# rwl/CSparse.py

Measured on AMD Instinct MI355X. Metric: cs_gaxpy achieved HBM GB/s (algorithmic bytes / time), 5M x 5M CSC, 64 nnz/col, higher is better.
Workload: dtype f64; 1 GPU; cs_gaxpy y += A x on G-rand: 5000000 x 5000000 CSC, 64 distinct rows per column drawn uniformly from [0, n), ascending (SURVEY 8d), int32 indices, fp64 values; one independent matrix per GPU; row_draw=uniform, n=5000000, nnz=320000000, kernel=gaxpy_tiled, plan_key_bytes=3, parallelism=independent matrices, 1 per GPU, no data-path collective

## Files before the change

csparse.py_amd/csrc/csx_gaxpy_tiled.hip:

```cpp
#include <cstdlib>

#include "csx_internal.h"

namespace csx {

constexpr int TL_WAVES = 4, TL_NG = 5;
constexpr int TL_GROUP = 256;
constexpr int TL_LDS_BYTES = 160 * 1024 - 256;
constexpr int TL_LDS_ROWS = TL_LDS_BYTES / 8 - 2;
typedef uint32_t u32x4 __attribute__((ext_vector_type(4)));
typedef double f64x2 __attribute__((ext_vector_type(2)));

__global__ __launch_bounds__(256) void k_tile_keys(int64_t nnz, const int32_t *__restrict__ Ai,
                                                   const int32_t *__restrict__ col, int rb_bits, int32_t row_block,
                                                   int32_t slab_cols, int32_t nslab, uint32_t *__restrict__ tile_id,
                                                   uint32_t *__restrict__ packed) {
    int64_t p = (int64_t)blockIdx.x * blockDim.x + threadIdx.x;
    if (p >= nnz) return;
    const uint32_t i = (uint32_t)Ai[p], j = (uint32_t)col[p];
    const uint32_t s = j / (uint32_t)slab_cols, lc = j - s * (uint32_t)slab_cols;
    const uint32_t b = i / (uint32_t)row_block, lr = i - b * (uint32_t)row_block;
    tile_id[p] = b * (uint32_t)nslab + s;
    packed[p] = (lc << rb_bits) | lr;
}

__global__ __launch_bounds__(256) void k_padded_lengths(int64_t ntiles, const int32_t *__restrict__ sptr,
                                                        int32_t *__restrict__ ngroups) {
    int64_t t = (int64_t)blockIdx.x * blockDim.x + threadIdx.x;
    if (t < ntiles) ngroups[t] = (sptr[t + 1] - sptr[t] + TL_GROUP - 1) / TL_GROUP;
}

__global__ __launch_bounds__(256) void k_group_info(int64_t ntiles, int32_t nslab, const int32_t *__restrict__ sptr,
                                                    const int32_t *__restrict__ gptr, uint32_t *__restrict__ info) {
    int64_t t = (int64_t)blockIdx.x * blockDim.x + threadIdx.x;
    if (t >= ntiles) return;
    const int32_t len = sptr[t + 1] - sptr[t];
    const uint32_t slab = (uint32_t)(t % nslab);
    int32_t g = gptr[t];
    for (int32_t left = len; left > 0; left -= TL_GROUP, g++) info[g] = (slab << 9) | (uint32_t)min(left, TL_GROUP);
}

__global__ __launch_bounds__(256) void k_interleave(int64_t nnz, const uint32_t *__restrict__ stid,
                                                    const int32_t *__restrict__ sptr, const int32_t *__restrict__ gptr,
                                                    const uint32_t *__restrict__ skey, const double *__restrict__ sval,
                                                    uint32_t *__restrict__ okey, double *__restrict__ oval) {
    int64_t q = (int64_t)blockIdx.x * blockDim.x + threadIdx.x;
    if (q >= nnz) return;
    const uint32_t t = stid[q];
    const int32_t e = (int32_t)(q - sptr[t]);
    const int32_t g = e / TL_GROUP, w = e % TL_GROUP;
    const int64_t gbase = ((int64_t)gptr[t] + g) * TL_GROUP;
    const int l = w & 63, k = w >> 6;
    if (okey) okey[gbase + l * 4 + k] = skey[q];
    oval[gbase + (k >> 1) * 128 + l * 2 + (k & 1)] = sval[q];
}

__global__ __launch_bounds__(256) void k_run_span(int64_t nnz, const uint32_t *__restrict__ stid,
                                                  const int32_t *__restrict__ sptr, const uint32_t *__restrict__ skey,
                                                  int rb_bits, int *too_wide) {
    int64_t q = (int64_t)blockIdx.x * blockDim.x + threadIdx.x;
    if (q >= nnz) return;
    const int32_t e = (int32_t)(q - sptr[stid[q]]);
    const int64_t first = q - (e & 63);
    if ((skey[q] >> rb_bits) - (skey[first] >> rb_bits) >= 512u) *too_wide = 1;
}

__global__ __launch_bounds__(256) void k_interleave24(int64_t nnz, const uint32_t *__restrict__ stid,
                                                      const int32_t *__restrict__ sptr, const int32_t *__restrict__ gptr,
                                                      const uint32_t *__restrict__ skey, int rb_bits,
                                                      uint8_t *__restrict__ okey, uint32_t *__restrict__ obase) {
    int64_t q = (int64_t)blockIdx.x * blockDim.x + threadIdx.x;
    if (q >= nnz) return;
    const uint32_t t = stid[q];
    const int32_t e = (int32_t)(q - sptr[t]);
    const int32_t g = e / TL_GROUP, w = e % TL_GROUP;
    const int l = w & 63, k = w >> 6;
    const uint32_t rmask = (1u << rb_bits) - 1u;
    const uint32_t col = skey[q] >> rb_bits, col0 = skey[q - l] >> rb_bits;
    const uint32_t v = (skey[q] & rmask) | ((col - col0) << 15);
    const int64_t gg = (int64_t)gptr[t] + g;
    uint8_t *o = okey + gg * (TL_GROUP * 3) + l * 12 + k * 3;
    o[0] = (uint8_t)v;
    o[1] = (uint8_t)(v >> 8);
    o[2] = (uint8_t)(v >> 16);
    if (l == 0) obase[gg * 4 + k] = col;
}

__global__ __launch_bounds__(256) void k_fill_key24(uint8_t *p, int64_t nslots, uint32_t v) {
    int64_t i = (int64_t)blockIdx.x * blockDim.x + threadIdx.x;
    const int64_t stride = (int64_t)gridDim.x * blockDim.x;
    for (; i < nslots; i += stride) {
        p[3 * i] = (uint8_t)v;
        p[3 * i + 1] = (uint8_t)(v >> 8);
        p[3 * i + 2] = (uint8_t)(v >> 16);
    }
}

__global__ __launch_bounds__(256) void k_fill_keys(uint32_t *p, int64_t n, uint32_t v) {
    int64_t i = (int64_t)blockIdx.x * blockDim.x + threadIdx.x;
    const int64_t stride = (int64_t)gridDim.x * blockDim.x;
    for (; i < n; i += stride) p[i] = v;
}

struct GroupRegs {
    u32x4 kk;
    u32x4 base;
    f64x2 v0, v1;
    uint32_t info;
};

template <bool NT, bool K24>
__device__ __forceinline__ GroupRegs load_group_t(const uint32_t *__restrict__ key, const double *__restrict__ val,
                                                  const uint32_t *__restrict__ info, const uint32_t *__restrict__ base,
                                                  int32_t g, int lane) {
    GroupRegs r;
    const int64_t gb = (int64_t)g * TL_GROUP;
    if (K24) {
        const uint32_t *kp = key + (int64_t)g * (TL_GROUP * 3 / 4) + 3 * lane;
        const uint32_t ka = __builtin_nontemporal_load(kp), kb = __builtin_nontemporal_load(kp + 1),
                       kc = __builtin_nontemporal_load(kp + 2);
        r.kk.x = ka & 0xFFFFFFu;
        r.kk.y = (ka >> 24) | ((kb & 0xFFFFu) << 8);
        r.kk.z = (kb >> 16) | ((kc & 0xFFu) << 16);
        r.kk.w = kc >> 8;
        r.base = *reinterpret_cast<const u32x4 *>(base + 4 * (int64_t)g);
        r.v0 = __builtin_nontemporal_load(reinterpret_cast<const f64x2 *>(val + gb + 2 * lane));
        r.v1 = __builtin_nontemporal_load(reinterpret_cast<const f64x2 *>(val + gb + 128 + 2 * lane));
    } else if (NT) {
        r.kk = __builtin_nontemporal_load(reinterpret_cast<const u32x4 *>(key + gb + 4 * lane));
        r.v0 = __builtin_nontemporal_load(reinterpret_cast<const f64x2 *>(val + gb + 2 * lane));
        r.v1 = __builtin_nontemporal_load(reinterpret_cast<const f64x2 *>(val + gb + 128 + 2 * lane));
    } else {
        r.kk = *reinterpret_cast<const u32x4 *>(key + gb + 4 * lane);
        r.v0 = *reinterpret_cast<const f64x2 *>(val + gb + 2 * lane);
        r.v1 = *reinterpret_cast<const f64x2 *>(val + gb + 128 + 2 * lane);
    }
    r.info = info[g];
    return r;
}

template <int HOW>
__device__ __forceinline__ double load_x(const double *p) {
    if (HOW == 1) return __hip_atomic_load(p, __ATOMIC_RELAXED, __HIP_MEMORY_SCOPE_AGENT);
    if (HOW == 2) return __builtin_nontemporal_load(p);
    return *p;
}

template <int VARIANT, int NW, int NG, bool K24>
struct TiledStep {
    static constexpr bool GATHER = !(VARIANT & 1) || VARIANT >= 5, ATOMIC = VARIANT != 3;
    static constexpr bool STREAM_NT = VARIANT != 2;
    static constexpr uint32_t CMASK = VARIANT == 5 ? 32767u : (VARIANT == 4 ? 255u : 0xffffffffu);
    static constexpr int XLOAD = VARIANT == 6 ? 1 : 0;
    static constexpr bool RING = VARIANT == 7;

    static __device__ __forceinline__ void load_set(GroupRegs (&r)[NG], const uint32_t *__restrict__ key,
                                                    const double *__restrict__ val, const uint32_t *__restrict__ info,
                                                    const uint32_t *__restrict__ base, int32_t g, int32_t g0,
                                                    int32_t gend, int lane) {
#pragma unroll
        for (int j = 0; j < NG; j++) {
            int32_t gg = g + j * NW < gend ? g + j * NW : gend - 1;
            if (RING) gg = g0 + ((gg - g0) & 31);
            r[j] = load_group_t<STREAM_NT, K24>(key, val, info, base, gg, lane);
        }
    }

    static __device__ __forceinline__ void step(GroupRegs (&cur)[NG], GroupRegs (&nxt)[NG], double *ytile,
                                                const uint32_t *__restrict__ key, const double *__restrict__ val,
                                                const uint32_t *__restrict__ info, const uint32_t *__restrict__ base,
                                                const double *__restrict__ x, int32_t &g, int32_t g0, int32_t gend,
                                                int lane, int rb_bits, uint32_t rmask, int32_t slab_cols, double &sink) {
        double xv[NG][4];
#pragma unroll
        for (int j = 0; j < NG; j++) {
            xv[j][0] = xv[j][1] = xv[j][2] = xv[j][3] = 1.0;
            if (GATHER && (j == 0 || g + j * NW < gend)) {
                const double *xs = x + (int64_t)(cur[j].info >> 9) * slab_cols;
                if (K24) {
                    xv[j][0] = load_x<XLOAD>(xs + ((cur[j].base.x + (cur[j].kk.x >> 15)) & CMASK));
                    xv[j][1] = load_x<XLOAD>(xs + ((cur[j].base.y + (cur[j].kk.y >> 15)) & CMASK));
                    xv[j][2] = load_x<XLOAD>(xs + ((cur[j].base.z + (cur[j].kk.z >> 15)) & CMASK));
                    xv[j][3] = load_x<XLOAD>(xs + ((cur[j].base.w + (cur[j].kk.w >> 15)) & CMASK));
                } else {
                    xv[j][0] = load_x<XLOAD>(xs + ((cur[j].kk.x >> rb_bits) & CMASK));
                    xv[j][1] = load_x<XLOAD>(xs + ((cur[j].kk.y >> rb_bits) & CMASK));
                    xv[j][2] = load_x<XLOAD>(xs + ((cur[j].kk.z >> rb_bits) & CMASK));
                    xv[j][3] = load_x<XLOAD>(xs + ((cur[j].kk.w >> rb_bits) & CMASK));
                }
            }
        }
        load_set(nxt, key, val, info, base, g + NG * NW, g0, gend, lane);
#pragma unroll
        for (int j = 0; j < NG; j++) {
            if (j == 0 || g + j * NW < gend) {
                if (ATOMIC) {
                    unsafeAtomicAdd(&ytile[cur[j].kk.x & rmask], cur[j].v0.x * xv[j][0]);
                    unsafeAtomicAdd(&ytile[cur[j].kk.y & rmask], cur[j].v0.y * xv[j][1]);
                    unsafeAtomicAdd(&ytile[cur[j].kk.z & rmask], cur[j].v1.x * xv[j][2]);
                    unsafeAtomicAdd(&ytile[cur[j].kk.w & rmask], cur[j].v1.y * xv[j][3]);
                } else {
                    sink += cur[j].v0.x * xv[j][0] + cur[j].v0.y * xv[j][1] + cur[j].v1.x * xv[j][2] +
                            cur[j].v1.y * xv[j][3] +
                            (double)((cur[j].kk.x ^ cur[j].kk.y ^ cur[j].kk.z ^ cur[j].kk.w) & 1u);
                }
            }
        }
        g += NG * NW;
    }
};

template <int VARIANT, int NW, int NG, bool K24>
__global__ __launch_bounds__(64 * NW) void k_gaxpy_tiled(const int32_t *__restrict__ rb_gptr,
                                                         const uint32_t *__restrict__ group_info,
                                                         const uint32_t *__restrict__ tile_key,
                                                         const uint32_t *__restrict__ tile_base,
                                                         const double *__restrict__ tile_val,
                                                         const double *__restrict__ x, double *__restrict__ y,
                                                         int32_t m, int32_t nrb, int32_t row_block,
                                                         int32_t slab_cols, int rb_bits) {
    extern __shared__ __attribute__((aligned(16))) double ytile[];
    typedef TiledStep<VARIANT, NW, NG, K24> S;
    const uint32_t rmask = K24 ? 0x7FFFu : (1u << rb_bits) - 1u;
    const int lane = threadIdx.x & 63, wave = threadIdx.x >> 6;
    double sink = 0.0;
    for (int32_t rb = blockIdx.x; rb < nrb; rb += gridDim.x) {
        const int64_t row0 = (int64_t)rb * row_block;
        const int32_t rows = (int32_t)((row0 + row_block <= m) ? row_block : (m - row0));
        for (int k = threadIdx.x; k < rows; k += 64 * NW) ytile[k] = y[row0 + k];
        __syncthreads();
        const int32_t gend = rb_gptr[rb + 1];
        const int32_t g0 = rb_gptr[rb];
        int32_t g = g0 + wave;
        if (g < gend) {
            GroupRegs A[NG], B[NG];
            S::load_set(A, tile_key, tile_val, group_info, tile_base, g, g0, gend, lane);
            for (;;) {
                S::step(A, B, ytile, tile_key, tile_val, group_info, tile_base, x, g, g0, gend, lane, rb_bits, rmask, slab_cols, sink);
                if (g >= gend) break;
                S::step(B, A, ytile, tile_key, tile_val, group_info, tile_base, x, g, g0, gend, lane, rb_bits, rmask, slab_cols, sink);
                if (g >= gend) break;
            }
        }
        __syncthreads();
        if (!S::ATOMIC && sink == 12345.678) ytile[0] = sink;
        for (int k = threadIdx.x; k < rows; k += 64 * NW) y[row0 + k] = ytile[k];
        __syncthreads();
    }
}

__global__ __launch_bounds__(256) void k_rb_group_ptr(int32_t nrb, int32_t nslab, const int32_t *__restrict__ gptr,
                                                      int32_t *__restrict__ rb_gptr) {
    int64_t b = (int64_t)blockIdx.x * blockDim.x + threadIdx.x;
    if (b <= nrb) rb_gptr[b] = gptr[(int64_t)b * nslab];
}

static int gaxpy_tiled_pick_shape(Csc *A);

int gaxpy_tiled_prepare(Csc *A) {
    if (A->tiled) return CSX_OK;
    if (!A->x) return CSX_EINVAL;
    hipStream_t s = ctx().stream;
    const int32_t nwg = ctx().cus > 0 ? ctx().cus : 256;
    const int32_t cap = TL_LDS_ROWS;
    int32_t rounds = 1;
    int32_t row_block;
    for (;;) {
        const int64_t nrb_try = (int64_t)nwg * rounds;
        row_block = (int32_t)(((int64_t)A->m + nrb_try - 1) / nrb_try);
        if (row_block <= cap) break;
        rounds++;
    }
    if (row_block < 1) row_block = 1;
    const int32_t nrb = (int32_t)(((int64_t)A->m + row_block - 1) / row_block);
    int rb_bits = 1;
    while ((1 << rb_bits) <= row_block) rb_bits++;
    double slab_kb = 1024.0;
#ifdef CSX_ABLATION
    if (const char *e = std::getenv("CSX_TILED_SLAB_KB")) slab_kb = std::atof(e) >= 8.0 ? std::atof(e) : slab_kb;
#endif
    int64_t slab_cols = (int64_t)(slab_kb * 1024 / 8);
    const int64_t max_cols_key = 1ll << (32 - rb_bits);
    if (slab_cols > max_cols_key) slab_cols = max_cols_key;
    if (slab_cols > A->n) slab_cols = A->n > 0 ? A->n : 1;
    int32_t nslab = (int32_t)(((int64_t)A->n + slab_cols - 1) / slab_cols);
    if (nslab < 1) nslab = 1;
    const int64_t ntiles = (int64_t)nrb * nslab;
    if (ntiles > 0x3fffffffll || nslab >= (1 << 22)) return CSX_EINVAL;

    std::unique_ptr<TiledPlan> t(new TiledPlan());
    t->rb_bits = rb_bits;
    t->row_block = row_block;
    t->nrb = nrb;
    t->nslab = nslab;
    t->slab_cols = (int32_t)slab_cols;
    {
        DevBuf<int32_t> col, sptr, gptr;
        DevBuf<uint32_t> tid, packed, stid, skey;
        DevBuf<double> sval;
        int64_t ngroups = 0;
        CSX_TRY(col.alloc((size_t)A->nnz));
        CSX_TRY(tid.alloc((size_t)A->nnz));
        CSX_TRY(packed.alloc((size_t)A->nnz));
        CSX_TRY(stid.alloc((size_t)A->nnz));
        CSX_TRY(skey.alloc((size_t)A->nnz));
        CSX_TRY(sval.alloc((size_t)A->nnz));
        CSX_TRY(sptr.alloc((size_t)ntiles + 1));
        CSX_TRY(gptr.alloc((size_t)ntiles + 1));
        CSX_TRY(t->tile_ptr.alloc((size_t)nrb + 1));
        CSX_TRY(expand_columns(A->p, A->n, A->nnz, col));
        if (A->nnz > 0) {
            int64_t blocks = ((int64_t)A->nnz + 255) / 256;
            hipLaunchKernelGGL(k_tile_keys, dim3((unsigned)blocks), dim3(256), 0, s, (int64_t)A->nnz, A->i, col, rb_bits,
                               row_block, t->slab_cols, t->nslab, tid, packed);
            CSX_LAUNCH_CHECK();
        }
        CSX_TRY(stable_sort_by_key(tid, packed, A->x, A->nnz, (uint32_t)ntiles, stid, skey, sval));
        CSX_TRY(boundaries_from_sorted(stid, A->nnz, (int32_t)ntiles, sptr));
        const unsigned tb = (unsigned)((ntiles + 256) / 256);
        hipLaunchKernelGGL(k_padded_lengths, dim3(tb), dim3(256), 0, s, ntiles, sptr, gptr);
        CSX_TRY(scan_exclusive_i32(gptr, gptr, ntiles, &ngroups));
        bool k24 = false;
        if (ngroups > 0 && rb_bits <= 15 && ctx().opt.gaxpy_keys24) {
            DevBuf<int> flag;
            int h = 1;
            CSX_TRY(flag.alloc(1));
            (void)hipMemsetAsync(flag, 0, sizeof(int), s);
            hipLaunchKernelGGL(k_run_span, dim3((unsigned)(((int64_t)A->nnz + 255) / 256)), dim3(256), 0, s, (int64_t)A->nnz,
                               stid, sptr, skey, rb_bits, flag);
            CSX_HIP(hipMemcpyAsync(&h, flag, sizeof(int), hipMemcpyDeviceToHost, s));
            CSX_HIP(hipStreamSynchronize(s));
            k24 = h == 0;
        }
        t->ngroups = ngroups;
        CSX_TRY(t->tile_len.alloc((size_t)ngroups));
        if (!k24) CSX_TRY(t->tile_key.alloc((size_t)ngroups * TL_GROUP));
        if (k24) CSX_TRY(t->tile_key24.alloc((size_t)ngroups * TL_GROUP * 3 + 16));
        if (k24) CSX_TRY(t->tile_base.alloc((size_t)ngroups * 4));
        CSX_TRY(t->tile_val.alloc((size_t)ngroups * TL_GROUP));
        if (ngroups > 0) {
            if (k24) {
                hipLaunchKernelGGL(k_fill_key24, dim3(2048), dim3(256), 0, s, t->tile_key24, (int64_t)ngroups * TL_GROUP,
                                   (uint32_t)row_block);
                (void)hipMemsetAsync(t->tile_base, 0, (size_t)ngroups * 4 * sizeof(uint32_t), s);
            } else {
                hipLaunchKernelGGL(k_fill_keys, dim3(2048), dim3(256), 0, s, t->tile_key, (int64_t)ngroups * TL_GROUP,
                                   (uint32_t)row_block);
            }
            (void)hipMemsetAsync(t->tile_val, 0, (size_t)ngroups * TL_GROUP * sizeof(double), s);
            hipLaunchKernelGGL(k_group_info, dim3(tb), dim3(256), 0, s, ntiles, nslab, sptr, gptr, (uint32_t *)t->tile_len.get());
            hipLaunchKernelGGL(k_interleave, dim3((unsigned)(((int64_t)A->nnz + 255) / 256)), dim3(256), 0, s,
                               (int64_t)A->nnz, stid, sptr, gptr, skey, sval, t->tile_key, t->tile_val);
            if (k24)
                hipLaunchKernelGGL(k_interleave24, dim3((unsigned)(((int64_t)A->nnz + 255) / 256)), dim3(256), 0, s,
                                   (int64_t)A->nnz, stid, sptr, gptr, skey, rb_bits, t->tile_key24, t->tile_base);
        }
        hipLaunchKernelGGL(k_rb_group_ptr, dim3((unsigned)((nrb + 256) / 256)), dim3(256), 0, s, nrb, nslab, gptr,
                           t->tile_ptr);
        CSX_LAUNCH_CHECK();
        CSX_HIP(hipStreamSynchronize(s));
    }
    A->tiled = std::move(t);
#ifndef CSX_ABLATION
    if (ctx().opt.gaxpy_tune_shape) CSX_TRY(gaxpy_tiled_pick_shape(A));
#endif
    return CSX_OK;
}

constexpr int TL_NSHAPES = 4;
static int gaxpy_tiled_launch(const Csc *A, const double *x, double *y, int shape);

static int gaxpy_tiled_pick_shape(Csc *A) {
    TiledPlan *t = A->tiled.get();
    if ((int64_t)A->nnz < (int64_t)1 << 24) return CSX_OK;
    hipStream_t s = ctx().stream;
    DevBuf<double> x, y;
    if (x.alloc((size_t)A->n) != CSX_OK || y.alloc((size_t)A->m) != CSX_OK) return CSX_OK;
    CSX_HIP(hipMemsetAsync(x, 0, (size_t)A->n * sizeof(double), s));
    CSX_HIP(hipMemsetAsync(y, 0, (size_t)A->m * sizeof(double), s));
    hipEvent_t e0, e1;
    CSX_HIP(hipEventCreate(&e0));
    CSX_HIP(hipEventCreate(&e1));
    int best = 0;
    int st = CSX_OK;
    for (int round = 0; round < 2 && st == CSX_OK; round++)
        for (int sh = 0; sh < TL_NSHAPES && st == CSX_OK; sh++) {
            if (round == 0) st = gaxpy_tiled_launch(A, x, y, sh);
            if (st != CSX_OK) break;
            (void)hipEventRecord(e0, s);
            for (int rep = 0; rep < 3 && st == CSX_OK; rep++) st = gaxpy_tiled_launch(A, x, y, sh);
            (void)hipEventRecord(e1, s);
            if (hipEventSynchronize(e1) != hipSuccess) st = CSX_ERUNTIME;
            float ms = 0.f;
            (void)hipEventElapsedTime(&ms, e0, e1);
            ms /= 3;
            if (round == 0 || ms < t->shape_ms[sh]) t->shape_ms[sh] = ms;
        }
    (void)hipEventDestroy(e0);
    (void)hipEventDestroy(e1);
    if (st != CSX_OK) return st;
    for (int sh = 1; sh < TL_NSHAPES; sh++)
        if (t->shape_ms[sh] < t->shape_ms[best]) best = sh;
    t->shape = best;
    return CSX_OK;
}

int gaxpy_tiled_shape(const TiledPlan *t) {
    const int forced = ctx().opt.gaxpy_shape;
    if (forced >= 0 && forced < TL_NSHAPES) return forced;
    return t->shape >= 0 && t->shape < TL_NSHAPES ? t->shape : 0;
}

int gaxpy_tiled_run(const Csc *A, const double *x, double *y) {
    return gaxpy_tiled_launch(A, x, y, gaxpy_tiled_shape(A->tiled.get()));
}

int gaxpy_tiled_group_counts(const TiledPlan *t, std::vector<int32_t> &groups) {
    std::vector<int32_t> ptr((size_t)t->nrb + 1);
    hipStream_t s = ctx().stream;
    CSX_HIP(hipMemcpyAsync(ptr.data(), t->tile_ptr, ptr.size() * sizeof(int32_t), hipMemcpyDeviceToHost, s));
    CSX_HIP(hipStreamSynchronize(s));
    groups.resize((size_t)t->nrb);
    for (int32_t b = 0; b < t->nrb; b++) groups[b] = ptr[b + 1] - ptr[b];
    return CSX_OK;
}

static int gaxpy_tiled_launch(const Csc *A, const double *x, double *y, int shape) {
    const TiledPlan *t = A->tiled.get();
    hipStream_t s = ctx().stream;
    const size_t lds = (((size_t)(t->row_block + 1) * sizeof(double)) + 15) & ~(size_t)15;
    const int32_t nwg = ctx().cus > 0 ? ctx().cus : 256;
    const unsigned grid = (unsigned)(t->nrb < nwg ? t->nrb : nwg);
#define CSX_TILED_LAUNCH_K(V, NW, NG, K24)                                                                           \
    {                                                                                                                \
        CSX_HIP(hipFuncSetAttribute(reinterpret_cast<const void *>(&k_gaxpy_tiled<V, NW, NG, K24>),                  \
                                    hipFuncAttributeMaxDynamicSharedMemorySize, TL_LDS_BYTES));                      \
        hipLaunchKernelGGL((k_gaxpy_tiled<V, NW, NG, K24>), dim3(grid), dim3(64 * NW), lds, s, t->tile_ptr,          \
                           (const uint32_t *)t->tile_len.get(),                                                      \
                           K24 ? reinterpret_cast<const uint32_t *>(t->tile_key24.get()) : t->tile_key.get(),        \
                           t->tile_base,                                                                             \
                           t->tile_val, x, y, A->m, t->nrb, t->row_block, t->slab_cols, t->rb_bits);                 \
    }
#define CSX_TILED_LAUNCH(V, NW, NG)                                                                                  \
    {                                                                                                                \
        if (t->tile_key24) CSX_TILED_LAUNCH_K(V, NW, NG, true) else CSX_TILED_LAUNCH_K(V, NW, NG, false)             \
    }
#ifdef CSX_ABLATION
    int code = 0;
    if (const char *e = std::getenv("CSX_TILED_VARIANT")) code = std::atoi(e);
    const int v = code % 100, nw = (code / 100) % 100 ? (code / 100) % 100 : TL_WAVES, ng = code / 10000 ? code / 10000 : TL_NG;
#define CSX_V(V)                                             \
    if (v == V) {                                            \
        if (nw == 16 && ng == 2) CSX_TILED_LAUNCH(V, 16, 2)  \
        else if (nw == 4 && ng == 5) CSX_TILED_LAUNCH(V, 4, 5) \
        else if (nw == 2 && ng == 10) CSX_TILED_LAUNCH(V, 2, 10) \
        else return CSX_EINVAL;                              \
    } else
    if (v == 0) {
        if (nw == 16 && ng == 1) CSX_TILED_LAUNCH(0, 16, 1)
        else if (nw == 16 && ng == 2) CSX_TILED_LAUNCH(0, 16, 2)
        else if (nw == 12 && ng == 2) CSX_TILED_LAUNCH(0, 12, 2)
        else if (nw == 12 && ng == 4) CSX_TILED_LAUNCH(0, 12, 4)
        else if (nw == 8 && ng == 2) CSX_TILED_LAUNCH(0, 8, 2)
        else if (nw == 8 && ng == 3) CSX_TILED_LAUNCH(0, 8, 3)
        else if (nw == 8 && ng == 4) CSX_TILED_LAUNCH(0, 8, 4)
        else if (nw == 4 && ng == 4) CSX_TILED_LAUNCH(0, 4, 4)
        else if (nw == 4 && ng == 5) CSX_TILED_LAUNCH(0, 4, 5)
        else if (nw == 4 && ng == 6) CSX_TILED_LAUNCH(0, 4, 6)
        else if (nw == 2 && ng == 6) CSX_TILED_LAUNCH(0, 2, 6)
        else if (nw == 2 && ng == 7) CSX_TILED_LAUNCH(0, 2, 7)
        else if (nw == 2 && ng == 8) CSX_TILED_LAUNCH(0, 2, 8)
        else if (nw == 2 && ng == 9) CSX_TILED_LAUNCH(0, 2, 9)
        else if (nw == 2 && ng == 10) CSX_TILED_LAUNCH(0, 2, 10)
        else if (nw == 2 && ng == 12) CSX_TILED_LAUNCH(0, 2, 12)
        else if (nw == 1 && ng == 10) CSX_TILED_LAUNCH(0, 1, 10)
        else if (nw == 1 && ng == 12) CSX_TILED_LAUNCH(0, 1, 12)
        else if (nw == 3 && ng == 5) CSX_TILED_LAUNCH(0, 3, 5)
        else if (nw == 3 && ng == 6) CSX_TILED_LAUNCH(0, 3, 6)
        else if (nw == 3 && ng == 7) CSX_TILED_LAUNCH(0, 3, 7)
        else if (nw == 3 && ng == 8) CSX_TILED_LAUNCH(0, 3, 8)
        else if (nw == 5 && ng == 4) CSX_TILED_LAUNCH(0, 5, 4)
        else if (nw == 6 && ng == 3) CSX_TILED_LAUNCH(0, 6, 3)
        else if (nw == 4 && ng == 7) CSX_TILED_LAUNCH(0, 4, 7)
        else return CSX_EINVAL;
    } else
    CSX_V(1) CSX_V(2) CSX_V(3) CSX_V(4) CSX_V(5) CSX_V(6) CSX_V(7) return CSX_EINVAL;
#undef CSX_V
    (void)shape;
#else
    switch (shape) {
        case 1: CSX_TILED_LAUNCH(0, 2, 10) break;
        case 2: CSX_TILED_LAUNCH(0, 8, 4) break;
        case 3: CSX_TILED_LAUNCH(0, 2, 8) break;
        default: CSX_TILED_LAUNCH(0, TL_WAVES, TL_NG) break;
    }
#endif
#undef CSX_TILED_LAUNCH
#undef CSX_TILED_LAUNCH_K
    CSX_LAUNCH_CHECK();
    return CSX_OK;
}

}
```

Baseline: 5072 GB/s.

## Zero-fill LDS y tile and fold y read into pipelined drain

Instead of loading y from global memory into the LDS tile before the accumulation phase, the default path fills the tile with -0.0 after the first group loads have been issued, so the y read no longer stalls the start of each row block. During the drain, y is read from global memory in double-buffered register chunks and added to the LDS partial sums before the store. The aim is to overlap y traffic with the accumulate and store work and to remove a serialized global-load-then-barrier step. The old behaviour stays available as variant 8. The cost is extra register use and a more complex tail path.

```diff
diff --git a/csparse.py_amd/csrc/csx_gaxpy_tiled.hip b/csparse.py_amd/csrc/csx_gaxpy_tiled.hip
--- a/csparse.py_amd/csrc/csx_gaxpy_tiled.hip
+++ b/csparse.py_amd/csrc/csx_gaxpy_tiled.hip
@@ -10,6 +10,7 @@
 constexpr int TL_LDS_ROWS = TL_LDS_BYTES / 8 - 2;
 typedef uint32_t u32x4 __attribute__((ext_vector_type(4)));
 typedef double f64x2 __attribute__((ext_vector_type(2)));
+constexpr int TL_DRAIN_U = 4;
 
 __global__ __launch_bounds__(256) void k_tile_keys(int64_t nnz, const int32_t *__restrict__ Ai,
                                                    const int32_t *__restrict__ col, int rb_bits, int32_t row_block,
@@ -210,6 +211,38 @@
     }
 };
 
+template <int NT>
+__device__ __forceinline__ void tl_fill(double *ytile, int32_t row_block) {
+    f64x2 *yt2 = reinterpret_cast<f64x2 *>(ytile);
+    const f64x2 mz = {-0.0, -0.0};
+    for (int k = threadIdx.x; k < (row_block + 2) >> 1; k += NT) yt2[k] = mz;
+}
+
+template <int NT, int U>
+__device__ __forceinline__ void tl_drain_load(double (&r)[U], const double *yblk, int32_t k0, int32_t rows) {
+#pragma unroll
+    for (int u = 0; u < U; u++) {
+        const int32_t k = k0 + u * NT;
+        r[u] = yblk[k < rows ? k : rows - 1];
+    }
+}
+
+template <int NT, int U, bool WHOLE>
+__device__ __forceinline__ void tl_drain_store(const double (&r)[U], double *yblk, const double *ytile, int32_t k0,
+                                               int32_t rows) {
+    double t[U];
+#pragma unroll
+    for (int u = 0; u < U; u++) {
+        const int32_t k = k0 + u * NT;
+        t[u] = ytile[(WHOLE || k < rows) ? k : rows - 1];
+    }
+#pragma unroll
+    for (int u = 0; u < U; u++) {
+        const int32_t k = k0 + u * NT;
+        if (WHOLE || k < rows) yblk[k] = r[u] + t[u];
+    }
+}
+
 template <int VARIANT, int NW, int NG, bool K24>
 __global__ __launch_bounds__(64 * NW) void k_gaxpy_tiled(const int32_t *__restrict__ rb_gptr,
                                                          const uint32_t *__restrict__ group_info,
@@ -221,30 +254,69 @@
                                                          int32_t slab_cols, int rb_bits) {
     extern __shared__ __attribute__((aligned(16))) double ytile[];
     typedef TiledStep<VARIANT, NW, NG, K24> S;
+    constexpr bool Y_HEAD = VARIANT == 8;
+    constexpr int NT = 64 * NW, U = TL_DRAIN_U;
     const uint32_t rmask = K24 ? 0x7FFFu : (1u << rb_bits) - 1u;
     const int lane = threadIdx.x & 63, wave = threadIdx.x >> 6;
     double sink = 0.0;
     for (int32_t rb = blockIdx.x; rb < nrb; rb += gridDim.x) {
         const int64_t row0 = (int64_t)rb * row_block;
         const int32_t rows = (int32_t)((row0 + row_block <= m) ? row_block : (m - row0));
-        for (int k = threadIdx.x; k < rows; k += 64 * NW) ytile[k] = y[row0 + k];
-        __syncthreads();
         const int32_t gend = rb_gptr[rb + 1];
         const int32_t g0 = rb_gptr[rb];
         int32_t g = g0 + wave;
-        if (g < gend) {
-            GroupRegs A[NG], B[NG];
+        const bool busy = __builtin_amdgcn_readfirstlane(g < gend);
+        GroupRegs A[NG], B[NG];
+        if (Y_HEAD) {
+            for (int k = threadIdx.x; k < rows; k += NT) ytile[k] = y[row0 + k];
+            __syncthreads();
+        }
+        if (busy) {
             S::load_set(A, tile_key, tile_val, group_info, tile_base, g, g0, gend, lane);
+            if (!Y_HEAD) {
+                tl_fill<NT>(ytile, row_block);
+                __syncthreads();
+            }
             for (;;) {
                 S::step(A, B, ytile, tile_key, tile_val, group_info, tile_base, x, g, g0, gend, lane, rb_bits, rmask, slab_cols, sink);
                 if (g >= gend) break;
                 S::step(B, A, ytile, tile_key, tile_val, group_info, tile_base, x, g, g0, gend, lane, rb_bits, rmask, slab_cols, sink);
                 if (g >= gend) break;
             }
-        }
-        __syncthreads();
-        if (!S::ATOMIC && sink == 12345.678) ytile[0] = sink;
-        for (int k = threadIdx.x; k < rows; k += 64 * NW) y[row0 + k] = ytile[k];
+        } else if (!Y_HEAD) {
+            tl_fill<NT>(ytile, row_block);
+            __syncthreads();
+        }
+        if (Y_HEAD) {
+            __syncthreads();
+            if (!S::ATOMIC && sink == 12345.678) ytile[0] = sink;
+            for (int k = threadIdx.x; k < rows; k += NT) y[row0 + k] = ytile[k];
+        } else {
+            int32_t tid = (int32_t)threadIdx.x;
+            asm volatile("" : "+v"(tid));
+            double *yblk = y + row0;
+            constexpr int CH = NT * U;
+            double ca[U], cb[U];
+            tl_drain_load<NT, U>(ca, yblk, tid, rows);
+            __syncthreads();
+            if (!S::ATOMIC && sink == 12345.678) ytile[0] = sink;
+            for (int32_t base = 0;;) {
+                if (base + CH > rows) {
+                    if (base < rows) tl_drain_store<NT, U, false>(ca, yblk, ytile, base + tid, rows);
+                    break;
+                }
+                tl_drain_load<NT, U>(cb, yblk, base + CH + tid, rows);
+                tl_drain_store<NT, U, true>(ca, yblk, ytile, base + tid, rows);
+                base += CH;
+                if (base + CH > rows) {
+                    if (base < rows) tl_drain_store<NT, U, false>(cb, yblk, ytile, base + tid, rows);
+                    break;
+                }
+                tl_drain_load<NT, U>(ca, yblk, base + CH + tid, rows);
+                tl_drain_store<NT, U, true>(cb, yblk, ytile, base + tid, rows);
+                base += CH;
+            }
+        }
         __syncthreads();
     }
 }
@@ -455,6 +527,13 @@
         else if (nw == 4 && ng == 5) CSX_TILED_LAUNCH(V, 4, 5) \
         else if (nw == 2 && ng == 10) CSX_TILED_LAUNCH(V, 2, 10) \
         else return CSX_EINVAL;                              \
+    } else
+    if (v == 8) {
+        if (nw == 4 && ng == 5) CSX_TILED_LAUNCH(8, 4, 5)
+        else if (nw == 2 && ng == 10) CSX_TILED_LAUNCH(8, 2, 10)
+        else if (nw == 8 && ng == 4) CSX_TILED_LAUNCH(8, 8, 4)
+        else if (nw == 2 && ng == 8) CSX_TILED_LAUNCH(8, 2, 8)
+        else return CSX_EINVAL;
     } else
     if (v == 0) {
         if (nw == 16 && ng == 1) CSX_TILED_LAUNCH(0, 16, 1)
```

Measured after the change: 5177 GB/s (median of 6 runs). +2.1%, better.
